# PolyChord/PolyChordLite

Hardware: AMD Instinct MI355X
Metric: likelihood evals/sec, 20D Gaussian nlive=2000 (higher is better)
Workload: dtype f64; 1 GPU; configs[1]: 20-D Gaussian, nlive=2000, num_repeats=40, one full run per step; batch_chains=1000, parallelism=repeat-sharded x1, mode=one run at a time per GPU; R runs in step: roofline.in_step

## Files before the change

include/polychord_hip.h:

```cpp
#ifndef POLYCHORD_HIP_H
#define POLYCHORD_HIP_H
#include <stdbool.h>
#ifdef __cplusplus
extern "C" {
#endif


typedef double (*polychord_loglike_fn)(double *theta, int nDims, double *phi, int nDerived);
typedef void (*polychord_prior_fn)(double *cube, double *theta, int nDims);
typedef void (*polychord_dumper_fn)(int ndead, int nlive, int npars, double *live, double *dead,
                                    double *logweights, double logZ, double logZerr);

void polychord_c_interface(
    polychord_loglike_fn loglikelihood, polychord_prior_fn prior, polychord_dumper_fn dumper,
    int nlive, int num_repeats, int nprior, int nfail, bool do_clustering, int feedback,
    double precision_criterion, double logzero, int max_ndead, double boost_posterior,
    bool posteriors, bool equals, bool cluster_posteriors, bool write_resume, bool write_paramnames,
    bool read_resume, bool write_stats, bool write_live, bool write_dead, bool write_prior,
    bool maximise, double compression_factor, bool synchronous, int nDims, int nDerived,
    char *base_dir, char *file_root, int nGrade, double *grade_frac, int *grade_dims, int n_nlives,
    double *loglikes, int *nlives, int seed, int *comm);

void polychord_c_interface_ini(polychord_loglike_fn loglikelihood, void (*setup_loglikelihood)(void),
                               char *inifile, int *comm);
// ... 229 lines not shown
int  pchip_run_in_step(const pchip_settings *s, const pchip_like *like, const pchip_prior *prior, int nseeds, const int *seeds,
                       int ndevices, const int *devices, int max_in_flight, int want_rows, pchip_result *results, pchip_merged *merged);

typedef struct pchip_comm pchip_comm;
#define PCHIP_COMM_ID_BYTES 128
int  pchip_comm_get_id(char *id128);
int  pchip_comm_create(const char *id128, int nranks, int rank, int device, pchip_comm **out);
void pchip_comm_destroy(pchip_comm *c);
int  pchip_comm_merge(pchip_comm *c, const pchip_result *run, double logzero, int nDims, int nDerived, int want_rows,
                      pchip_merged *out);
int  pchip_comm_merge_many(pchip_comm *c, const pchip_result *runs, int nruns, double logzero, int nDims, int nDerived, int want_rows,
                           pchip_merged *out);
typedef int (*pchip_allgather_fn)(void *user, const void *send, void *recv, unsigned long bytes);
int  pchip_comm_create_with(pchip_allgather_fn all_gather, void *user, int nranks, int rank, int device, pchip_comm **out);
const char *pchip_comm_library(void);

int  pchip_slice_chains(const pchip_settings *s, const pchip_like *like, const pchip_prior *prior,
                        unsigned batch, int nchains, const double *seeds, const double *chol,
                        double contour, double *babies_out, double *nhats_out, int *nlike_out);
#define PCHIP_NO_SUCH_PATH 64
int  pchip_directions(const pchip_settings *s, const pchip_like *like, const pchip_prior *prior, unsigned batch, int nchains,
                      const double *seeds, const double *chol, int path, double *nhat_out, double *nhat_w_out,
                      double *nhat_Ms_out, double *ch_My_out, int *has_Ms, double *raw_out, int nrows, int nbases);
int  pchip_prior_transform(const pchip_prior *prior, int nDims, int n, const double *cube, double *theta, int device);
int  pchip_update_factors(const pchip_settings *s, int ncluster, int nlive, const double *live, const int *live_cluster,
                          int nph, const double *phantom, const double *ph_logL, const int *ph_cluster, const double *threshold,
                          const double *shift, int path, double *cov, double *chol, int *count, double *shift_out, int *chol_suspect);
typedef struct {
    int ncluster, nlive, nph;
    const double *live, *live_logL; const int *live_cluster;
    const double *phantom, *ph_logL; const int *ph_cluster;
} pchip_cluster_in;
typedef struct {
    int maxc, nsplit_cap, scratch_cap;
    int ncluster, nsplit, levels, scratch_n;
    int *live_cluster, *live_pos, *cl_list;
    int *cl_n, *imin_slot, *ph_count; unsigned *cl_uid;
    double *logLp, *lse_ref, *lse_sum, *logXp, *logZp, *logZXp, *logZp2, *logZpXp;
    double *XpXq;
    int *ph_cluster;
    unsigned *split_child, *split_parent; double *split_logfrac;
    double *init;
    double *scratch_Sm; int *scratch_knn, *scratch_lab;
} pchip_cluster_out;
int  pchip_cluster_update(const pchip_settings *s, int nsets, const pchip_cluster_in *in, pchip_cluster_out *out, int path);

// ... 12 lines not shown
```

polychordlite_amd/_ctypes_api.py:

```python
import ctypes as C
import os

import numpy as np

_HERE = os.path.dirname(os.path.abspath(__file__))
LIB_PATH = os.environ.get("PCHIP_LIB") or os.path.join(_HERE, "libpolychord_hip.so")

LOGLIKE_FN = C.CFUNCTYPE(C.c_double, C.POINTER(C.c_double), C.c_int, C.POINTER(C.c_double), C.c_int)
PRIOR_FN = C.CFUNCTYPE(None, C.POINTER(C.c_double), C.POINTER(C.c_double), C.c_int)
DUMPER_FN = C.CFUNCTYPE(None, C.c_int, C.c_int, C.c_int, C.POINTER(C.c_double), C.POINTER(C.c_double),
                        C.POINTER(C.c_double), C.c_double, C.c_double)

LIKE_CALLBACK, LIKE_GAUSSIAN, LIKE_RASTRIGIN, LIKE_TWIN_GAUSSIAN, LIKE_CORR_GAUSSIAN, LIKE_SOURCE = range(6)
KERNEL_CLASSES = ("k_nhats", "k_slice", "k_consume", "k_apply", "k_clean", "k_covmats", "k_bases_side")
LIKE_KINDS = {"gaussian": LIKE_GAUSSIAN, "rastrigin": LIKE_RASTRIGIN, "twin_gaussian": LIKE_TWIN_GAUSSIAN,
              "corr_gaussian": LIKE_CORR_GAUSSIAN, "source": LIKE_SOURCE}


class Settings(C.Structure):
    _fields_ = [("nDims", C.c_int), ("nDerived", C.c_int), ("nlive", C.c_int), ("num_repeats", C.c_int),
                ("nprior", C.c_int), ("nfail", C.c_int), ("do_clustering", C.c_int),
                ("precision_criterion", C.c_double), ("logzero", C.c_double), ("max_ndead", C.c_int),
                ("boost_posterior", C.c_double), ("posteriors", C.c_int), ("equals", C.c_int),
                ("cluster_posteriors", C.c_int), ("compression_factor", C.c_double), ("n_nlives", C.c_int),
# ... 474 lines not shown
    ch = np.ascontiguousarray(chol, dtype=np.float64)
    assert ch.shape == (D, D) and sd.shape[1] == 2 * D + settings.nDerived + 2
    nch = sd.shape[0]
    if settings.nGrade > 1:
        off = np.concatenate([[0], np.cumsum([settings.grade_dims[g] for g in range(settings.nGrade)])[:-1]])
        reps = [settings.grade_repeats[g] for g in range(settings.nGrade)]
    else:
        off, reps = [0], [settings.num_repeats]
    nr = int(sum(reps))
    nb = int(sum(-(-r // (D - o)) for r, o in zip(reps, off)))
    nhat = np.full((nch, nr, D), np.nan); w = np.full((nch, nr), np.nan)
    Ms = np.full((nch, nr, D), np.nan); My = np.full((nch, D), np.nan); raw = np.full((nch, nb, D, D), np.nan)
    has = C.c_int(0)
    rc = lib.pchip_directions(C.byref(settings), C.byref(like), C.byref(prior), batch, nch, dptr(sd), dptr(ch), path, dptr(nhat), dptr(w),
                              dptr(Ms), dptr(My), C.byref(has), dptr(raw), nr, nb)
    if rc == NO_SUCH_PATH:
        return None
    if rc != 0:
        msg = lib.polychord_hip_last_error()
        raise RuntimeError(f"pchip_directions failed with code {rc}" + (": " + msg.decode(errors="replace") if rc == 1 and msg else ""))
    return dict(nhat=nhat, nhat_w=w, nhat_Ms=Ms if has.value else None, ch_My=My if has.value else None, raw=raw if path else None)


def maximum_dict(m, nDims, nDerived):
    n = nDims + nDerived
    pt = lambda p: np.ctypeslib.as_array(p, shape=(n,)).copy() if p else None
    return dict(status=[int(v) for v in m.status], cluster=[int(v) for v in m.cluster], niter=[int(v) for v in m.niter], neval=[int(v) for v in m.neval],
                max_logl=m.max_logl, max_point=pt(m.max_point), max_post=m.max_post, logl_at_post=m.logl_at_post, post_point=pt(m.post_point),
                logl_mean=m.logl_mean if m.has_mean else None, mean_point=pt(m.mean_point) if m.has_mean else None)


def _maximum_out(lib, m, rc, who, nDims, nDerived, write):
    try:
        if rc != 0 and not (rc == 1 and m.max_point and (m.status[0] or m.status[1])):
            msg = lib.polychord_hip_last_error()
            raise RuntimeError(f"{who} failed with code {rc}" + (": " + msg.decode(errors="replace") if msg else ""))
        if write is not None and lib.pchip_maximum_write(C.byref(m), nDims, nDerived, str(write).encode()) != 0:
            raise RuntimeError(f"pchip_maximum_write({write}) failed")
        return maximum_dict(m, nDims, nDerived)
    finally:
        lib.pchip_maximum_free(C.byref(m))


def maximise_device(settings, like, prior, run, max_iter=0, write=None):
    lib = load()
    live = np.ascontiguousarray(run["live"], dtype=np.float64)
# ... 129 lines not shown
```

polychordlite_amd/csrc/pc_dev.h:

```cpp
#pragma once
#ifndef __HIPCC_RTC__
#include <hip/hip_runtime.h>
#include <stdint.h>
#else
using __hip_internal::uint32_t; using __hip_internal::uint64_t; using __hip_internal::int32_t; using __hip_internal::int64_t;
typedef unsigned long uintptr_t;
#endif

#define PC_WAVE 64
#define PC_SLICE_STRIDE 128
enum { PC_DOM_LIVEGEN = 0, PC_DOM_SEED = 1, PC_DOM_NHAT = 2, PC_DOM_SHUFFLE = 3, PC_DOM_SLICE = 4,
       PC_DOM_PHANTOM = 5, PC_DOM_POST = 6, PC_DOM_SEQ = 0xFFFF };
enum { PC_LIKE_CALLBACK = 0, PC_LIKE_GAUSSIAN = 1, PC_LIKE_RASTRIGIN = 2, PC_LIKE_TWIN_GAUSSIAN = 3,
       PC_LIKE_CORR_GAUSSIAN = 4, PC_LIKE_SOURCE = 5 };
#define PC_SRC_MAX_DERIVED 32

#define PC_HUGE 1.7976931348623157e308
#define PC_LOG_TWO_PI 1.8378770664093453
#define PC_TWO_PI 6.283185307179586

struct u32x4 { uint32_t x, y, z, w; };

__device__ __forceinline__ u32x4 philox4x32_10(uint32_t c0, uint32_t c1, uint32_t c2, uint32_t c3,
                                                uint32_t k0, uint32_t k1)
// ... 96 lines not shown
__device__ inline double pc_inv_normal_tail(double p)
{
    const double c[8] = { 1.42343711074968357734e+00, 4.63033784615654529590e+00,
        5.76949722146069140550e+00, 3.64784832476320460504e+00, 1.27045825245236838258e+00,
        2.41780725177450611770e-01, 2.27238449892691845833e-02, 7.74545014278341407640e-04 };
    const double d[8] = { 1.0, 2.05319162663775882187e+00, 1.67638483018380384940e+00,
        6.89767334985100004550e-01, 1.48103976427480074590e-01, 1.51986665636164571966e-02,
        5.47593808499534494600e-04, 1.05075007164441684324e-09 };
    const double e[8] = { 6.65790464350110377720e+00, 5.46378491116411436990e+00,
        1.78482653991729133580e+00, 2.96560571828504891230e-01, 2.65321895265761230930e-02,
        1.24266094738807843860e-03, 2.71155556874348757815e-05, 2.01033439929228813265e-07 };
    const double f[8] = { 1.0, 5.99832206555887937690e-01, 1.36929880922735805310e-01,
        1.48753612908506148525e-02, 7.86869131145613259100e-04, 1.84631831751005468180e-05,
        1.42151175831644588870e-07, 2.04426310338993978564e-15 };
    const double q = p - 0.5;
    double r = (q < 0.0) ? p : 1.0 - p;
    r = sqrt(-log(r));
    double v;
    if (r <= 5.0) { r -= 1.6; v = poly8(c, r) / poly8(d, r); }
    else          { r -= 5.0; v = poly8(e, r) / poly8(f, r); }
    return (q < 0.0) ? -v : v;
}

__device__ __forceinline__ double pc_logaddexp(double a, double b)
{
    const bool ab = a > b;
    const double hi = ab ? a : b, d = ab ? b - a : a - b;
    if (d < -37.0) return hi;
    return hi + log(exp(d) + 1.0);
}

__device__ __forceinline__ void pc_lds_barrier() { asm volatile("s_waitcnt lgkmcnt(0)\n\ts_barrier" ::: "memory"); }

#define PC_DPP_XOR1 0xB1
#define PC_DPP_XOR2 0x4E
#define PC_DPP_HALF_MIRROR 0x141
#define PC_DPP_MIRROR 0x140
template <int CTRL>
constexpr bool pc_dpp_full = CTRL < 0x100 || CTRL == PC_DPP_HALF_MIRROR || CTRL == PC_DPP_MIRROR;
template <int CTRL>
__device__ __forceinline__ int dpp_i32(int v) { return __builtin_amdgcn_update_dpp(0, v, CTRL, 0xF, 0xF, pc_dpp_full<CTRL>); }
template <int CTRL>
__device__ __forceinline__ double dpp_f64(double v)
{
    const int lo = dpp_i32<CTRL>(__double2loint(v));
    const int hi = dpp_i32<CTRL>(__double2hiint(v));
// ... 98 lines not shown
```

polychordlite_amd/csrc/pc_engine.hip:

```cpp
#include "pc_state.h"
#include "pc_resume.h"
#include "pc_prior_table.h"
#include "pc_launch.h"
#include "pc_plan.h"
#include <cstdio>
#include <cstdlib>
#include <cstring>
#include <cstdarg>
#include <cstdint>
#include <new>
#include <cmath>
#include <vector>
#include <memory>
#include <string>
#include <chrono>
#include <algorithm>
#include <map>
#include <unordered_map>
#include <atomic>
#include <mutex>
#include <thread>
#include <functional>
#include <exception>
#include <ucontext.h>
// ... 1601 lines not shown
    }
    bool enqueue_nursery()
    {
        unsigned &batch = r_batch; int &nursery_left = r_nursery_left;
        if (S.pool) {
            if (pool_cursor + (long long)B * S.nr > S.Pcap) pool_compact();
            S.pool_base = (int)pool_cursor; S.pool_rows = B * S.nr; S.babies = S.phantom + (size_t)pool_cursor * S.nT;
            pool_cursor += (long long)B * S.nr;
        }
        {
            hipEvent_t e0 = kt.begin(KT_NHATS);
            const PcNurseryChoice ch = pc_choose_nursery(plan, nursery_facts(batch));
            pc_count(path, ch);
            pc_count_step(path, ch);
            int bases_seq = 0;
            switch (ch.bases) {
            case PC_BASES_READY: case PC_BASES_PART1: case PC_BASES_PART1_STEP: {
                RawSlot &rs = ring[batch % raw_depth];
                S.nhat_raw = raw_buf[batch % raw_depth];
                if (ch.bases == PC_BASES_READY) { if (!rs.waited) HIPCHK(hipStreamWaitEvent(st, rs.ready, 0)); bases_seq = rs.co_seq; }
                else {
                    if (rs.valid) HIPCHK(hipStreamWaitEvent(st, rs.ready, 0));
                    if (ch.bases == PC_BASES_PART1_STEP) co->rec(rec_bases(S, batch, B));
                    else (void)pc_launch_nhats_part(&S, batch, B, 1, st, ch.packed ? 1 : 0);
                }
                rs.valid = false;
                if (ch.part2) { if (co) { co->flush(); co->wait_next(); } (void)pc_launch_nhats_part(&S, batch, B, 2, st, 0); }
                break;
            }
            case PC_BASES_NHATS_G: co->rec(rec_nhats_g(S, batch, B)); break;
            case PC_BASES_WHOLE:
                if (co) co->flush();
                if (pc_launch_nhats(&S, batch, B, st)) { std::fprintf(stderr, "polychord_hip: nDims unsupported\n"); r_rc = 3; return false; }
                break;
            }
            kt.end(KT_NHATS, e0);
            hipEvent_t e1 = kt.begin(KT_SLICE);
            switch (ch.sampler) {
            case PC_SAMPLER_CALLBACK:
                if (co) co->flush();
                if (dev_batch) slice_device(batch); else slice_callback(batch);
                if (stop.load(std::memory_order_relaxed)) { r_rc = 5; return false; }
                break;
            case PC_SAMPLER_LANE: { Cohort::Rec r = rec_slice(S, batch, B, bases_seq); r.note = co ? &step_note : nullptr; (void)stage(r); break; }
            case PC_SAMPLER_WAVE_STEP: co->rec(rec_slice_g(S, batch, B, ch.fused, ch.fused ? bases_seq : 0, &step_note)); break;
            case PC_SAMPLER_WAVE:
                if (co) { co->flush(); co->wait_next(); }
// ... 39 lines not shown
        if (!ev_presort_a) { ev_presort_a = hpool().get_sync_event(); ev_presort_b = hpool().get_sync_event(); }
        HIPCHK(hipEventRecord(ev_presort_a, st)); HIPCHK(hipStreamWaitEvent(st_side, ev_presort_a, 0));
        if (pc_launch_sort_live(&S, st_side) != 0) return;
        HIPCHK(hipEventRecord(ev_presort_b, st_side));
        presorted = true;
    }
    void side_prefetch(unsigned cur)
    {
        const unsigned batch = cur;
        {
        ensure_side();
        const bool side_free = pc_env().side_free || (S.D > 64 && !pc_env().side_ordered);
        RawSlot &cur = ring[batch % raw_depth];
        if (side_free) { HIPCHK(hipEventRecord(cur.consumed, st)); cur.used = true; }
        if (!side_free) { HIPCHK(hipEventRecord(ev_main, st)); HIPCHK(hipStreamWaitEvent(st_side, ev_main, 0)); }
        const unsigned xmax = batch + (unsigned)raw_depth - (side_free ? 0u : 1u);
        for (unsigned x = batch + 1; x <= xmax; ++x) {
            RawSlot &rs = ring[x % raw_depth];
            if (rs.valid && rs.batch == x && rs.B == B) continue;
            if (rs.valid) continue;
            if (rs.used) HIPCHK(hipStreamWaitEvent(st_side, rs.consumed, 0));
            PcState S1 = S; S1.nhat_raw = raw_buf[x % raw_depth];
            hipEvent_t es = kt.begin_on(KT_SIDE, st_side);
            (void)pc_launch_nhats_part(&S1, x, B, 1, st_side, (cfg.ablate & PC_ABL_BASES_PACKED) ? 1 : 0);
            kt.end_on(KT_SIDE, es, st_side);
            HIPCHK(hipEventRecord(rs.ready, st_side));
            rs.valid = true; rs.batch = x; rs.B = B; rs.waited = false;
        }
    }
    }

    PcContractFacts contract_facts(int nursery_left) const
    {
        PcContractFacts f{};
        f.ncluster = h_ctl->ncluster; f.nursery_left = nursery_left;
        f.in_step = co != nullptr; f.cohort_general = cohort_general_ok();
        f.nn_lists = S.nn_list && !pc_env().nn_lists_off; f.nn_valid = S.nn_valid != 0;
        f.cl_fits = f.ncluster > 1 && pc_consume_cl_fits(&S, f.ncluster) != 0;
        f.clp_fits = f.cl_fits && pc_consume_clp_fits(&S, f.ncluster) != 0;
        return f;
    }
    bool round_enqueue()
    {
        unsigned &batch = r_batch; bool &sort_valid = r_sort_valid; int &nursery_left = r_nursery_left;
        {
            if (h_ctl->status == PC_ST_DONE) return false;
            if (h_ctl->status == PC_ST_ERROR) { std::fprintf(stderr, "polychord_hip: device error %d\n", h_ctl->error); r_rc = 2; return false; }
// ... 431 lines not shown
    try {
        E.setup(c, *like, *prior);
        PcState &S = E.S;
        const int nT = S.nT, D = S.D, nr = S.nr, nb = S.nb_total;
        if (nrows != nr || nbases != nb) {
            pc_abi_set_last_error("pchip_directions: the caller's arrays are for another number of directions or bases than the settings give");
            rc = 1;
        } else if ((path != 0 && !pc_nhats_splittable(&S)) || (path == 2 && !pc_bases_t_ok(&S))) rc = PCHIP_NO_SUCH_PATH;
        if (has_Ms) *has_Ms = S.nhat_Ms != nullptr ? 1 : 0;
        if (rc == 0) {
            HIPCHK(hipMemcpy(S.live, seeds, sizeof(double) * (size_t)nchains * nT, hipMemcpyHostToDevice));
            std::vector<double> ll(nchains); std::vector<int> idn(nchains), zero(nchains, 0);
            for (int i = 0; i < nchains; ++i) { ll[i] = seeds[(size_t)i * nT + S.l0]; idn[i] = i; }
            const double contour = *std::min_element(ll.begin(), ll.end());
            HIPCHK(hipMemcpy(S.live_logL, ll.data(), sizeof(double) * nchains, hipMemcpyHostToDevice));
            HIPCHK(hipMemcpy(S.live_cluster, zero.data(), sizeof(int) * nchains, hipMemcpyHostToDevice));
            HIPCHK(hipMemcpy(S.live_pos, idn.data(), sizeof(int) * nchains, hipMemcpyHostToDevice));
            HIPCHK(hipMemcpy(S.cl_list, idn.data(), sizeof(int) * nchains, hipMemcpyHostToDevice));
            HIPCHK(hipMemcpy(S.cl_n, &nchains, sizeof(int), hipMemcpyHostToDevice));
            HIPCHK(hipMemcpy(S.logLp, &contour, sizeof(double), hipMemcpyHostToDevice));
            HIPCHK(hipMemcpy(S.chol, chol, sizeof(double) * D * D, hipMemcpyHostToDevice));
            S.seed_override = 1;
            if (path == 0) rc = pc_launch_nhats(&S, batch, nchains, E.st) ? PCHIP_NO_SUCH_PATH : 0;
            else rc = (pc_launch_nhats_part(&S, batch, nchains, 1, E.st, path == 2 ? 1 : 0) || pc_launch_nhats_part(&S, batch, nchains, 2, E.st, 0)) ? PCHIP_NO_SUCH_PATH : 0;
            HIPCHK(hipStreamSynchronize(E.st));
            HIPCHK(hipGetLastError());
        }
        if (rc == 0) {
            HIPCHK(hipMemcpy(nhat_out, S.nhat, sizeof(double) * (size_t)nchains * nr * D, hipMemcpyDeviceToHost));
            HIPCHK(hipMemcpy(nhat_w_out, S.nhat_w, sizeof(double) * (size_t)nchains * nr, hipMemcpyDeviceToHost));
            if (S.nhat_Ms && nhat_Ms_out) HIPCHK(hipMemcpy(nhat_Ms_out, S.nhat_Ms, sizeof(double) * (size_t)nchains * nr * D, hipMemcpyDeviceToHost));
            if (S.ch_My && ch_My_out) HIPCHK(hipMemcpy(ch_My_out, S.ch_My, sizeof(double) * (size_t)nchains * D, hipMemcpyDeviceToHost));
        }
        if (rc == 0 && path != 0) {
            const size_t blk = D <= 24 ? (size_t)D * D : D <= 32 ? (size_t)1024 : D <= 64 ? (size_t)4096 : (size_t)32 * 512;
            std::vector<double> raw((size_t)nchains * nb * blk);
            HIPCHK(hipMemcpy(raw.data(), S.nhat_raw, sizeof(double) * raw.size(), hipMemcpyDeviceToHost));
            for (size_t cb = 0; cb < (size_t)nchains * nb; ++cb) {
                const double *in = raw.data() + cb * blk;
                double *out = raw_out + cb * (size_t)D * D;
                for (int v = 0; v < D; ++v)
                    for (int d = 0; d < D; ++d) {
                        size_t at;
                        if (D <= 24) at = (size_t)v * D + d;
                        else if (D <= 64) at = (size_t)v * (D <= 32 ? 32 : 64) + d;
                        else { const int n = 2 * (d >> 3) + (d & 1), lk = (d & 7) >> 1; at = (size_t)n * 512 + 64 * (v >> 4) + 16 * lk + (v & 15); }
                        out[(size_t)v * D + d] = in[at];
                    }
            }
        }
    } catch (const EngineError &e) {
        std::fprintf(stderr, "polychord_hip: %s\n", e.msg.c_str());
        (void)hipGetLastError();
        rc = e.code;
    }
    E.destroy();
    return rc;
}

int pchip_prior_transform(const pchip_prior *prior, int nDims, int n, const double *cube, double *theta, int device)
{
    if (!prior || prior->kind != PCHIP_PRIOR_TABLE || n < 1 || !cube || !theta) { pc_abi_set_last_error("pchip_prior_transform: a prior table (kind 2) and n >= 1 points"); return 1; }
    PcPriorTable T;
    const std::string err = pc_prior_table_build(nDims, prior->table, prior->hyper, T);
    if (!err.empty()) { pc_abi_set_last_error(err.c_str()); return 1; }
    if (nDims > 256) return 3;
    int ndev = 0;
    if (hipGetDeviceCount(&ndev) != hipSuccess || ndev == 0) { (void)hipGetLastError(); std::fprintf(stderr, "polychord_hip: no HIP device available -- this engine has no CPU path\n"); return 2; }
    if (hipSetDevice(device >= 0 ? device % ndev : 0) != hipSuccess) return 2;
    const std::vector<double> tp = T.dev_par(); const std::vector<int> ti = T.dev_int();
    double *d_tp = nullptr, *d_c = nullptr, *d_t = nullptr; int *d_ti = nullptr;
    const size_t nb = sizeof(double) * (size_t)n * nDims;
// ... 605 lines not shown
```

polychordlite_amd/csrc/pc_launch.h:

```cpp
#pragma once
#include "pc_state.h"
#include "../../include/polychord_hip.h"
#include <cstddef>
#include <memory>
#include <vector>

struct PcSourceForm {
    long nterms;
    int nsums;
    long nquad;
    long nshared;
    int has_prior;
    long long ndata, ntail;
    int alive;
};

static inline size_t pc_quad_lds(const PcSourceForm &f) { return f.nquad > 0 ? sizeof(double) * 2 * (size_t)((f.nquad + 1) & ~1L) : 0; }

static inline size_t pc_front_lds(const PcSourceForm &f) { return pc_quad_lds(f) + (f.nshared > 0 ? sizeof(double) * 2 * (size_t)((f.nshared + 1) & ~1L) : 0); }

static inline int pc_slice_phi_lds(const PcState *S, const PcSourceForm &f)
{
    const size_t sh0 = sizeof(double) * ((size_t)S->D + S->nr) + 16, tb = sizeof(double) * (size_t)S->nr * (S->D + 1);
    const size_t sums = sizeof(double) * (size_t)S->nr * (size_t)f.nsums;
// ... 61 lines not shown
void pc_batch_callback_get(polychord_batch_fn *fn, void **user);
int pc_device_batch_registered(void);
int pc_fast_fits(const PcState *S);
int pc_launch_sort_live(const PcState *S, hipStream_t st);
int pc_launch_sort_live_many(const PcState *S, const PcManyRec *dR, int R, hipStream_t st);
int pc_launch_consume_fast(const PcState *S, int final_mode, hipStream_t st);
void pc_launch_ph_prepare(const PcState *S, hipStream_t st);
size_t pc_records_block_bytes(long long cap, int nT);
int pc_pack_lived_device(const double *dead, const double *logw, const double *entry, long long nd, int nT, double logzero, double *block, long long cap, long long *h_count, hipStream_t st);
int pc_par_fits(const PcState *S);
int pc_launch_consume_par(const PcState *S, hipStream_t st);
int pc_launch_consume_par_many(const PcState *S, const PcManyRec *dR, int R, hipStream_t st);
int pc_launch_par_accept(int n, const double *snap, int T, const double *cand, const unsigned char *valid, int serial, unsigned char *accept,
                         hipStream_t st);
int pc_launch_final_par(const PcState *S, hipStream_t st);
int pc_launch_final_par_split(const PcState *S, hipStream_t st);
int pc_launch_final_par_many(const PcManyRec *dR, int R, hipStream_t st);
int pc_rtc_launch(const PcState *S, const char *expr, dim3 grid, dim3 block, size_t sh, hipStream_t st, void **args);
const char *pc_rtc_error(void);
int pc_rtc_source_form(int id, PcSourceForm *f);
int pc_rtc_wanted(const PcState *S);
int pc_launch_generate_live(const PcState *S, int attempt0, int n, double *rows, double *rows_logL, hipStream_t st);
int pc_nhats_splittable(const PcState *S);
int pc_launch_nhats_part(const PcState *S, unsigned batch, int nchains, int part, hipStream_t st, int packed);
int pc_launch_nhats(const PcState *S, unsigned batch, int nchains, hipStream_t st);
int pc_slice_fusable(const PcState *S);
int pc_launch_slice_fused(const PcState *S, unsigned batch, int nchains, hipStream_t st);
int pc_launch_slice_many(const PcState *S, const PcManyRec *dR, int R, int nchains, int fused, hipStream_t st);
int pc_launch_slice_step(const PcState *S, const PcManyRec *dR, int R, int nchains, int fused, hipStream_t st);
int pc_launch_nhats_many(const PcState *S, const PcManyRec *dR, int R, int nchains, hipStream_t st);
int pc_launch_slice(const PcState *S, unsigned batch, int nchains, hipStream_t st);
int pc_launch_prior_transform(const PcState *S, int n, const double *cubes, double *thetas, hipStream_t st);
int pc_launch_source_eval(const PcState *S, int n, const double *thetas, double *logL, double *phi, hipStream_t st);
int pc_launch_source_prior_eval(const PcState *S, int n, const double *cubes, double *thetas, hipStream_t st);
int pc_launch_max_rank(const PcState *S, int n, const double *rows, double *val, hipStream_t st);
int pc_launch_maximise(const PcState *S, int nprob, const double *in, const int *hdr, long long max_iter, double *out, long long *outi, hipStream_t st);
int pc_max_choose_simplex(int nDims, int nTotal, double logzero, const double *live, const int *cluster, int nlive, const double *vals,
                          double *simplex, double *f);
void pc_maximum_alloc(pchip_maximum *m, int nDims, int nDerived);
int pc_bases_t_ok(const PcState *S);
int pc_launch_bases_t(const PcState *S, unsigned batch, int nchains, hipStream_t st);
int pc_launch_bases_t_many(const PcState *S, const PcManyRec *dR, int R, unsigned batch, int nchains, hipStream_t st);
int pc_slice_t_ok(const PcState *S, int ncluster);
int pc_launch_slice_t(const PcState *S, unsigned batch, int nchains, hipStream_t st);
int pc_launch_slice_t_many(const PcState *S, const PcManyRec *dR, int R, unsigned batch, int nchains, hipStream_t st);
int pc_update_fused_ok(const PcState *S, int nc);
// ... 14 lines not shown
```

polychordlite_amd/csrc/pc_sample.hip:

```cpp
#include "pc_state.h"
#ifndef __HIPCC_RTC__
#include <cstdlib>
#endif

template <int DPL>
struct LaneDims {
    double lo[DPL], span[DPL];
    double mean[DPL];
    bool on[DPL];
};

__device__ __forceinline__ double pc_box_theta(double lo, double span, double cube) { return lo + span * cube; }
#define PC_PT_SORTED (1u << 16)
#define PC_PT_PERMUTED (1u << 17)
#define PC_PT_ADAPTIVE (1u << 18)
#define PC_PT_LAYER (1u << 19)
template <int DPL>
struct LaneTable {
    int type[DPL], pos[DPL], len[DPL], hyp[DPL];
    int cnt[DPL], lay[DPL];
    double p0[DPL], p1[DPL], p2[DPL];
    unsigned mask;
};
template <int DPL, bool AD>
// ... 1141 lines not shown
        if (active && wanted) {
            double n0 = 0.0, n1 = 0.0;
            int d = 0;
            for (; d + 1 < D; d += 2) { n0 += mine[d] * mine[d]; n1 += mine[d + 1] * mine[d + 1]; }
            if (d < D) n0 += mine[d] * mine[d];
            const double w = sqrt(n0 + n1);
            Q[i] = 1.0 / w;
            S.nhat_w[(size_t)chain * nr + col] = w * 3.0;
        }
        __syncthreads();
        for (int r = 0; r < Dg && basis * Dg + r < nrg; ++r) {
            double *out = S.nhat + ((size_t)chain * nr + col0 + basis * Dg + r) * D;
            const double iw = Q[r];
            for (int d = tid; d < D; d += NT) out[d] = G[(size_t)r * DS + d] * iw;
        }
    }
#ifdef NHATS_DBG
    ncyc[5] = clock64();
    if (tid == 0 && blockIdx.x == 0 && blockIdx.y == 0) for (int x = 0; x < 5; ++x) S.ctl->dbg[x] += ncyc[x + 1] - ncyc[x];
#endif
#undef PC_DOT4
}

#define PC_BIG_NT 256
#define PC_BIG_P 16
__global__ __launch_bounds__(PC_BIG_NT) void k_nhats_big(PcState S, unsigned batch)
{
    __shared__ int sh[2];
    __shared__ double iwv[PC_BIG_NT];
    __shared__ double Pq[PC_BIG_P * PC_BIG_NT];
    __shared__ double pqq[PC_BIG_P];
    const int D = S.D, nr = S.nr, tid = threadIdx.x, chain = blockIdx.y, i = tid;
    int grade, basis;
    pc_grade_of_basis(S, blockIdx.x, grade, basis);
    const int off = pc_sel(S.g_off, grade), Dg = D - off, nrg = pc_sel(S.g_nr, grade), col0 = pc_sel(S.g_col0, grade);
    if (tid == 0) {
        int sel, slot;
        select_seed(S, batch, chain, sel, slot);
        sh[0] = sel; sh[1] = slot;
        if (blockIdx.x == 0) {
            S.ch_cluster[chain] = sel; S.ch_seed_slot[chain] = slot;
            S.ch_contour[chain] = S.logLp[sel];
            S.ch_epoch[chain] = S.ctl->admin_epoch;
            if (chain == 0) { S.ctl->i_nursery = gridDim.y; S.ctl->batch_id = batch; }
        }
    }
// ... 772 lines not shown
{
    const size_t sh = sizeof(double) * S->D + pc_front_lds(pc_state_form(S));
    const bool table = S->prior.kind >= 2;
    switch (pc_dpl(S->D) + (table ? 8 : 0)) {
    case 1: PC_LAUNCH((k_generate_live<1>), dim3(n), dim3(64), sh, st, *S, attempt0, rows, rows_logL); return 0;
    case 2: PC_LAUNCH((k_generate_live<2>), dim3(n), dim3(64), sh, st, *S, attempt0, rows, rows_logL); return 0;
    case 4: PC_LAUNCH((k_generate_live<4>), dim3(n), dim3(64), sh, st, *S, attempt0, rows, rows_logL); return 0;
    case 9: PC_LAUNCH((k_generate_live<1, 1>), dim3(n), dim3(64), sh, st, *S, attempt0, rows, rows_logL); return 0;
    case 10: PC_LAUNCH((k_generate_live<2, 1>), dim3(n), dim3(64), sh, st, *S, attempt0, rows, rows_logL); return 0;
    case 12: PC_LAUNCH((k_generate_live<4, 1>), dim3(n), dim3(64), sh, st, *S, attempt0, rows, rows_logL); return 0;
    }
    return 1;
}

extern "C" int pc_nhats_splittable(const PcState *S)
{
    const char *e = std::getenv("PC_NHATS_QUAD_MIN");
    if (S->D > 64 && S->D <= 128) return S->ngrade <= 1 && !S->seq_mode && S->nhat_raw != nullptr;
    if (S->D > 24 && S->D <= 64) return S->ngrade <= 1 && !S->seq_mode && S->nhat_raw != nullptr && (!e || std::atoi(e) <= 25);
    return S->D <= 24 && S->D < (e ? std::atoi(e) : 25) && !S->seq_mode && S->nhat_raw != nullptr;
}
static size_t pc_nhats_q_lds(int HV) { return sizeof(double) * (size_t)(2 + HV) * 4 * (HV + 2); }
static size_t pc_nhats_q32_lds(int D) { const int NR = ((D + 15) / 16) * 16; return sizeof(double) * (2 * 4 * 34 + (size_t)(NR + (NR <= 112 ? 32 : 16)) * 129); }
extern "C" int pc_launch_nhats_part(const PcState *S, unsigned batch, int nchains, int part, hipStream_t st, int packed)
{
    if (!pc_nhats_splittable(S)) return 1;
    const int D = S->D;
    dim3 grid(S->nb_total, nchains);
    if (D > 64) {
        if (part == 1) {
            static const bool panel_off = std::getenv("PC_BASIS_PANEL_OFF") != nullptr;
            const int nt1 = (D + 15) / 16;
            if (panel_off) hipLaunchKernelGGL((k_nhats_q<32, 1>), grid, dim3(512), sizeof(double) * 2 * 4 * 34, st, *S, batch);
            else if (nt1 <= 5) hipLaunchKernelGGL((k_basis<5>), grid, dim3(512), 0, st, *S, batch);
            else if (nt1 == 6) hipLaunchKernelGGL((k_basis<6>), grid, dim3(512), 0, st, *S, batch);
            else if (nt1 == 7) hipLaunchKernelGGL((k_basis<7>), grid, dim3(512), 0, st, *S, batch);
            else hipLaunchKernelGGL((k_basis<8>), grid, dim3(512), 0, st, *S, batch);
        }
        else {
            dim3 g2(S->nb_total * 2, nchains);
            const int nt = (D + 15) / 16;
            if (nt <= 5) hipLaunchKernelGGL((k_whiten<5>), g2, dim3(256), 0, st, *S, batch);
            else if (nt == 6) hipLaunchKernelGGL((k_whiten<6>), g2, dim3(256), 0, st, *S, batch);
            else if (nt == 7) hipLaunchKernelGGL((k_whiten<7>), g2, dim3(256), 0, st, *S, batch);
            else hipLaunchKernelGGL((k_whiten<8>), g2, dim3(256), 0, st, *S, batch);
        }
        return 0;
    }
    if (D > 24) {
        if (D <= 32) { if (part == 1) hipLaunchKernelGGL((k_nhats_q<8, 1>), grid, dim3(128), pc_nhats_q_lds(8), st, *S, batch); else hipLaunchKernelGGL((k_nhats_q<8, 2>), grid, dim3(128), pc_nhats_q_lds(8), st, *S, batch); }
        else { if (part == 1) hipLaunchKernelGGL((k_nhats_q<16, 1>), grid, dim3(256), pc_nhats_q_lds(16), st, *S, batch); else hipLaunchKernelGGL((k_nhats_q<16, 2>), grid, dim3(256), pc_nhats_q_lds(16), st, *S, batch); }
        return 0;
    }
    const size_t sh = sizeof(double) * ((size_t)(D + 8) * (D + 8) + 2 * 128) + 16;
    if (part == 1 && packed && pc_launch_bases_t(S, batch, nchains, st) == 0) return 0;
    if (part == 1) {
        if (D <= 8) hipLaunchKernelGGL((k_nhats<8, 64, 1>), grid, dim3(64), sh, st, *S, batch);
        else if (D <= 16) hipLaunchKernelGGL((k_nhats<16, 64, 1>), grid, dim3(64), sh, st, *S, batch);
        else hipLaunchKernelGGL((k_nhats<24, 64, 1>), grid, dim3(64), sh, st, *S, batch);
    } else {
        if (D <= 8) hipLaunchKernelGGL((k_nhats<8, 64, 2>), grid, dim3(64), sh, st, *S, batch);
        else if (D <= 16) hipLaunchKernelGGL((k_nhats<16, 64, 2>), grid, dim3(64), sh, st, *S, batch);
        else hipLaunchKernelGGL((k_nhats<24, 64, 2>), grid, dim3(64), sh, st, *S, batch);
    }
    return 0;
}

extern "C" int pc_launch_nhats(const PcState *S, unsigned batch, int nchains, hipStream_t st)
{
    const int D = S->D, nb = S->nb_total;
    dim3 grid(nb, nchains);
    static int quad_min = -1;
    if (quad_min < 0) { const char *e = std::getenv("PC_NHATS_QUAD_MIN"); quad_min = e ? std::atoi(e) : 25; }
    if (D >= quad_min) {
        if (D <= 32) hipLaunchKernelGGL((k_nhats_q<8>), grid, dim3(128), pc_nhats_q_lds(8), st, *S, batch);
        else if (D <= 64) hipLaunchKernelGGL((k_nhats_q<16>), grid, dim3(256), pc_nhats_q_lds(16), st, *S, batch);
        else if (D <= 128) {
            const size_t shq = pc_nhats_q32_lds(D);
// ... 249 lines not shown
```

polychordlite_amd/csrc/pc_slice_t.hip:

```cpp
#include "pc_state.h"
#include "pc_launch.h"
#include <cstdlib>

namespace {

struct Q3 { double a, b, c; };

template <int D>
struct TriMap {
    int aa[D * (D + 1) / 2], bb[D * (D + 1) / 2];
    constexpr TriMap() : aa{}, bb{} { int e = 0; for (int b = 0; b < D; ++b) for (int a = b; a < D; ++a) { aa[e] = a; bb[e] = b; ++e; } }
};

template <int DT, int LO, int N, class F>
__device__ __forceinline__ Q3 tree3(const F &leaf)
{
#pragma clang fp contract(off)
    if constexpr (LO >= DT) return Q3{0.0, 0.0, 0.0};
    else if constexpr (N == 1) return leaf(LO);
    else {
        const Q3 l = tree3<DT, LO, N / 2>(leaf);
        if constexpr (LO + N / 2 >= DT && N / 2 >= 16) return l;
        const Q3 r = tree3<DT, LO + N / 2, N / 2>(leaf);
        return Q3{l.a + r.a, l.b + r.b, l.c + r.c};
// ... 405 lines not shown
    const bool unit = S->prior.lo == nullptr && S->prior.hi == nullptr;
    static const bool help_off = std::getenv("PC_SLICE_T_HELP_OFF") != nullptr;
    static const long long help_env = std::getenv("PC_SLICE_T_HELP_MAX") ? std::atoll(std::getenv("PC_SLICE_T_HELP_MAX")) : -1;
    const long long help_max = help_env >= 0 ? help_env : 256LL * std::max<long long>(1, std::min<long long>(2, (long long)(156 * 1024) / (long long)shh));
    const bool help = dR && !help_off && shh <= 64 * 1024 && (long long)grid * R <= help_max;
    const size_t lds = help ? shh : sh;
#define PC_T_MANY(UNIT, HELP) { \
        if (lds > 48 * 1024) pc_need_dyn_lds((const void *)k_slice_t_many<DT, UNIT, HELP>, lds); \
        hipLaunchKernelGGL((k_slice_t_many<DT, UNIT, HELP>), dim3(grid, R), dim3(HELP ? 192 : 64), lds, st, dR, nchains, nrp); }
#define PC_T_ONE(UNIT) { \
        if (lds > 48 * 1024) pc_need_dyn_lds((const void *)k_slice_t<DT, UNIT>, lds); \
        hipLaunchKernelGGL((k_slice_t<DT, UNIT>), dim3(grid), dim3(64), lds, st, *S, batch, nchains, nrp); }
    if (help) { if (unit) PC_T_MANY(true, true) else PC_T_MANY(false, true) }
    else if (dR) { if (unit) PC_T_MANY(true, false) else PC_T_MANY(false, false) }
    else { if (unit) PC_T_ONE(true) else PC_T_ONE(false) }
#undef PC_T_ONE
#undef PC_T_MANY
}

}

namespace {

template <int D, bool FIRST_RIGHT>
__device__ __forceinline__ double dot4_same(const double (&a)[D])
{
#pragma clang fp contract(off)
    double pp[4];
#pragma unroll
    for (int k = 0; k < 4; ++k) {
        if (k >= D) pp[k] = 0.0;
        else if (k + 4 >= D) pp[k] = fma(a[k], a[k], 0.0);
        else if (FIRST_RIGHT && k == 0) pp[k] = fma(a[k + 4 < D ? k + 4 : 0], a[k + 4 < D ? k + 4 : 0], a[k] * a[k]);
        else pp[k] = fma(a[k], a[k], a[k + 4 < D ? k + 4 : 0] * a[k + 4 < D ? k + 4 : 0]);
    }
#pragma unroll
    for (int d = 8; d < D; ++d) pp[d & 3] = fma(a[d], a[d], pp[d & 3]);
    return (pp[0] + pp[1]) + (pp[2] + pp[3]);
}
template <int D>
__device__ __forceinline__ double dot4(const double (&a)[D], const double (&b)[D])
{
#pragma clang fp contract(off)
    double pp[4] = {0.0, 0.0, 0.0, 0.0};
#pragma unroll
    for (int d = 0; d < D; ++d) pp[d & 3] = fma(a[d], b[d], pp[d & 3]);
    return (pp[0] + pp[1]) + (pp[2] + pp[3]);
}

template <int DMAX>
__device__ __forceinline__ void bases_packed_body(const PcState &S, int nbases)
{
#pragma clang fp contract(off)
    extern __shared__ __attribute__((aligned(16))) char smem[];
    const int D = S.D, per = 64 / D;
    const int tid = threadIdx.x, sub = tid / D, i = tid - sub * D;
    const int g = blockIdx.x * per + sub;
    const bool active = sub < per && g < nbases;
    double *Q = (double *)smem + (size_t)(sub < per ? sub : 0) * 2 * DMAX;
    double v[DMAX];
    double *raw = S.nhat_raw + ((size_t)(active ? g : 0) * D + i) * D;
#pragma unroll
    for (int d = 0; d < DMAX; ++d) v[d] = (active && d < D) ? raw[d] : 0.0;
    {
        const double inrm = 1.0 / sqrt(dot4_same<DMAX, (DMAX <= 16)>(v));
#pragma unroll
        for (int d = 0; d < DMAX; ++d) v[d] = v[d] * inrm;
    }
    if (i == 0 && active) {
#pragma unroll
        for (int d = 0; d < DMAX; ++d) Q[d] = v[d];
    }
    __syncthreads();
    for (int j = 0; j < D; ++j) {
        const double *q = Q + (size_t)(j & 1) * DMAX;
        double qv[DMAX];
#pragma unroll
        for (int d = 0; d < DMAX; ++d) qv[d] = active ? q[d] : 0.0;
        const double qq = dot4_same<DMAX, false>(qv), dv = dot4<DMAX>(qv, v);
        if (i == j) {
            const double inrm = 1.0 / sqrt(qq);
#pragma unroll
            for (int d = 0; d < DMAX; ++d) v[d] = v[d] * inrm;
        } else if (active && i > j) {
            const double cproj = dv / qq;
#pragma unroll
            for (int d = 0; d < DMAX; ++d) v[d] = fma(-cproj, qv[d], v[d]);
            if (i == j + 1) {
                double *qn = Q + (size_t)((j + 1) & 1) * DMAX;
#pragma unroll
                for (int d = 0; d < DMAX; ++d) qn[d] = v[d];
            }
        }
        __syncthreads();
    }
    if (active) {
#pragma unroll
        for (int d = 0; d < DMAX; ++d) if (d < D) raw[d] = v[d];
    }
}
template <int DMAX>
__global__ __launch_bounds__(64) void k_bases_packed(PcState S, int nbases) { bases_packed_body<DMAX>(S, nbases); }
template <int DMAX>
__global__ __launch_bounds__(64) void k_bases_packed_many(const PcManyRec *R, int nbases) { bases_packed_body<DMAX>(pc_many_state(R, blockIdx.y), nbases); }

#define DEVT_CALLS 4
__device__ __forceinline__ void deviates_t_body(const PcState &S, unsigned batch, int nbases, int NC)
{
    __shared__ double qU[4][2 * DEVT_CALLS * 64];
    __shared__ int qA[4][2 * DEVT_CALLS * 64];
    const int D = S.D, DD = D * D, lane = threadIdx.x & 63, wv = threadIdx.x >> 6;
    const long long ncalls = (long long)nbases * NC;
    int qn = 0;
    auto put = [&](bool want, double u, int dst) {
        bool t = false;
        double x = 0.0;
        if (want) x = pc_inv_normal_central(u, t);
        if (want && !t) S.nhat_raw[dst] = x;
// ... 90 lines not shown
```

polychordlite_amd/csrc/pc_state.h:

```cpp
#pragma once
#include "pc_dev.h"

enum { PC_ST_RUNNING = 0, PC_ST_DONE = 1, PC_ST_UPDATE = 2, PC_ST_ERROR = 4 };
enum { PC_ERR_NONE = 0, PC_ERR_PHANTOM_CAP = 1, PC_ERR_DEAD_CAP = 2, PC_ERR_CLUSTER_CAP = 3, PC_ERR_NOSLOT = 4 };

enum { PC_ABL_FUNCTOR = 1 << 0, PC_ABL_NO_POOL = 1 << 1, PC_ABL_NO_DEFER = 1 << 2, PC_ABL_NO_FUSED_UPDATE = 1 << 3, PC_ABL_PAIR_SCANS = 1 << 4,
       PC_ABL_CONSUME_GENERAL = 1 << 5, PC_ABL_SLICE_LANE = 1 << 6, PC_ABL_BASES_PACKED = 1 << 7, PC_ABL_CL_END_AT_DEATH = 1 << 8,
       PC_ABL_KILLOFF_GENERAL = 1 << 9, PC_ABL_CONSUME_CL_SERIAL = 1 << 10, PC_ABL_RETIRED_11 = 1 << 11, PC_ABL_RETIRED_12 = 1 << 12,
       PC_ABL_NO_HELPER = 1 << 13, PC_ABL_QC_BY_CHAIN = 1 << 14, PC_ABL_RTC_BUILTINS = 1 << 15, PC_ABL_UPDATE_CHAIN = 1 << 16, PC_ABL_FLAG_LAUNCH = 1 << 17,
       PC_ABL_ACCEPT_SERIAL = 1 << 18, PC_ABL_TRACE_CHOL = 1 << 30 };

#define PC_MASK_WORDS 16

struct PcCtl {
    int status;
    int error;
    int i_nursery;
    int admin_epoch;
    int failures;
    int ncluster;
    int ncluster_dead;
    int ndead;
    int nphantom;
    int seg_hi, seg_lo;
    int cluster_deleted;
    unsigned batch_id;
    unsigned next_cluster_uid;
    long long nlike;
    long long niter;
    long long nlike_device;
    long long nlike_failed;
    double logZ, logZ2;
    double logX_last_update;
// ... 227 lines not shown
```

Before: 1.392 billion likelihood evals/s.

## Fuse nhat random generation and Gram-Schmidt into one wave-per-bases kernel

Adds k_nhats_w, which draws the Gaussian deviates for several bases straight into shared memory, resolves tail inverse-normal cases through a compacted queue, and runs the packed Gram-Schmidt on them in the same 64-thread block. It becomes the default part-1 path, replacing the generic k_nhats part-1 kernel unless the new ablation bit is set. The aim is to avoid the separate raw-deviate write and re-read and to raise occupancy through small packed blocks. The Gram-Schmidt body is moved into a shared macro, and a deck_records test entry point is added. It risks divergence in the ballot queue and adds extra record writes for the deck.

```diff
diff --git a/include/polychord_hip.h b/include/polychord_hip.h
--- a/include/polychord_hip.h
+++ b/include/polychord_hip.h
@@ -275,6 +275,7 @@
 int  pchip_directions(const pchip_settings *s, const pchip_like *like, const pchip_prior *prior, unsigned batch, int nchains,
                       const double *seeds, const double *chol, int path, double *nhat_out, double *nhat_w_out,
                       double *nhat_Ms_out, double *ch_My_out, int *has_Ms, double *raw_out, int nrows, int nbases);
+int  pchip_deck_records(const pchip_settings *s, const pchip_like *like, const pchip_prior *prior, unsigned batch, int nchains, int *records);
 int  pchip_prior_transform(const pchip_prior *prior, int nDims, int n, const double *cube, double *theta, int device);
 int  pchip_update_factors(const pchip_settings *s, int ncluster, int nlive, const double *live, const int *live_cluster,
                           int nph, const double *phantom, const double *ph_logL, const int *ph_cluster, const double *threshold,
diff --git a/polychordlite_amd/_ctypes_api.py b/polychordlite_amd/_ctypes_api.py
--- a/polychordlite_amd/_ctypes_api.py
+++ b/polychordlite_amd/_ctypes_api.py
@@ -520,6 +520,20 @@
     return dict(nhat=nhat, nhat_w=w, nhat_Ms=Ms if has.value else None, ch_My=My if has.value else None, raw=raw if path else None)
 
 
+def deck_records(settings, like, prior, batch, nchains, fill=-1):
+    lib = load()
+    lib.pchip_deck_records.argtypes = [C.POINTER(Settings), C.POINTER(Like), C.POINTER(Prior), C.c_uint, C.c_int, C.POINTER(C.c_int)]
+    lib.pchip_deck_records.restype = C.c_int
+    rec = np.full((nchains, 66), fill, dtype=np.int32)
+    rc = lib.pchip_deck_records(C.byref(settings), C.byref(like), C.byref(prior), batch, nchains, rec.ctypes.data_as(C.POINTER(C.c_int)))
+    if rc == NO_SUCH_PATH:
+        return None
+    if rc != 0:
+        msg = lib.polychord_hip_last_error()
+        raise RuntimeError(f"pchip_deck_records failed with code {rc}" + (": " + msg.decode(errors="replace") if rc == 1 and msg else ""))
+    return rec
+
+
 def maximum_dict(m, nDims, nDerived):
     n = nDims + nDerived
     pt = lambda p: np.ctypeslib.as_array(p, shape=(n,)).copy() if p else None
diff --git a/polychordlite_amd/csrc/pc_dev.h b/polychordlite_amd/csrc/pc_dev.h
--- a/polychordlite_amd/csrc/pc_dev.h
+++ b/polychordlite_amd/csrc/pc_dev.h
@@ -142,6 +142,59 @@
     return (q < 0.0) ? -v : v;
 }
 
+template <int D, bool FIRST_RIGHT>
+__device__ __forceinline__ double dot4_same(const double (&a)[D])
+{
+#pragma clang fp contract(off)
+    double pp[4];
+#pragma unroll
+    for (int k = 0; k < 4; ++k) {
+        if (k >= D) pp[k] = 0.0;
+        else if (k + 4 >= D) pp[k] = fma(a[k], a[k], 0.0);
+        else if (FIRST_RIGHT && k == 0) pp[k] = fma(a[k + 4 < D ? k + 4 : 0], a[k + 4 < D ? k + 4 : 0], a[k] * a[k]);
+        else pp[k] = fma(a[k], a[k], a[k + 4 < D ? k + 4 : 0] * a[k + 4 < D ? k + 4 : 0]);
+    }
+#pragma unroll
+    for (int d = 8; d < D; ++d) pp[d & 3] = fma(a[d], a[d], pp[d & 3]);
+    return (pp[0] + pp[1]) + (pp[2] + pp[3]);
+}
+template <int D>
+__device__ __forceinline__ double dot4(const double (&a)[D], const double (&b)[D])
+{
+#pragma clang fp contract(off)
+    double pp[4] = {0.0, 0.0, 0.0, 0.0};
+#pragma unroll
+    for (int d = 0; d < D; ++d) pp[d & 3] = fma(a[d], b[d], pp[d & 3]);
+    return (pp[0] + pp[1]) + (pp[2] + pp[3]);
+}
+#define PC_GS_PACKED(DMAX, v, Q, D, i, active) \
+    {    \
+        const double inrm = 1.0 / sqrt(dot4_same<DMAX, (DMAX <= 16)>(v)); \
+        _Pragma("unroll") for (int d = 0; d < DMAX; ++d) v[d] = v[d] * inrm; \
+    } \
+    if (i == 0 && active) { \
+        _Pragma("unroll") for (int d = 0; d < DMAX; ++d) Q[d] = v[d]; \
+    } \
+    __syncthreads(); \
+    for (int j = 0; j < D; ++j) {                                                \
+        const double *q = Q + (size_t)(j & 1) * DMAX; \
+        double qv[DMAX]; \
+        _Pragma("unroll") for (int d = 0; d < DMAX; ++d) qv[d] = active ? q[d] : 0.0; \
+        const double qq = dot4_same<DMAX, false>(qv), dv = dot4<DMAX>(qv, v); \
+        if (i == j) { \
+            const double inrm = 1.0 / sqrt(qq); \
+            _Pragma("unroll") for (int d = 0; d < DMAX; ++d) v[d] = v[d] * inrm; \
+        } else if (active && i > j) { \
+            const double cproj = dv / qq; \
+            _Pragma("unroll") for (int d = 0; d < DMAX; ++d) v[d] = fma(-cproj, qv[d], v[d]); \
+            if (i == j + 1) { \
+                double *qn = Q + (size_t)((j + 1) & 1) * DMAX; \
+                _Pragma("unroll") for (int d = 0; d < DMAX; ++d) qn[d] = v[d]; \
+            } \
+        } \
+        __syncthreads(); \
+    }
+
 __device__ __forceinline__ double pc_logaddexp(double a, double b)
 {
     const bool ab = a > b;
diff --git a/polychordlite_amd/csrc/pc_engine.hip b/polychordlite_amd/csrc/pc_engine.hip
--- a/polychordlite_amd/csrc/pc_engine.hip
+++ b/polychordlite_amd/csrc/pc_engine.hip
@@ -1647,7 +1647,7 @@
                 else {
                     if (rs.valid) HIPCHK(hipStreamWaitEvent(st, rs.ready, 0));
                     if (ch.bases == PC_BASES_PART1_STEP) co->rec(rec_bases(S, batch, B));
-                    else (void)pc_launch_nhats_part(&S, batch, B, 1, st, ch.packed ? 1 : 0);
+                    else (void)pc_launch_nhats_part(&S, batch, B, 1, st, pc_part1_kind(ch.packed, cfg.ablate));
                 }
                 rs.valid = false;
                 if (ch.part2) { if (co) { co->flush(); co->wait_next(); } (void)pc_launch_nhats_part(&S, batch, B, 2, st, 0); }
@@ -1733,7 +1733,7 @@
             if (rs.used) HIPCHK(hipStreamWaitEvent(st_side, rs.consumed, 0));
             PcState S1 = S; S1.nhat_raw = raw_buf[x % raw_depth];
             hipEvent_t es = kt.begin_on(KT_SIDE, st_side);
-            (void)pc_launch_nhats_part(&S1, x, B, 1, st_side, (cfg.ablate & PC_ABL_BASES_PACKED) ? 1 : 0);
+            (void)pc_launch_nhats_part(&S1, x, B, 1, st_side, pc_part1_kind((cfg.ablate & PC_ABL_BASES_PACKED) != 0, cfg.ablate));
             kt.end_on(KT_SIDE, es, st_side);
             HIPCHK(hipEventRecord(rs.ready, st_side));
             rs.valid = true; rs.batch = x; rs.B = B; rs.waited = false;
@@ -2211,7 +2211,7 @@
             HIPCHK(hipMemcpy(S.chol, chol, sizeof(double) * D * D, hipMemcpyHostToDevice));
             S.seed_override = 1;
             if (path == 0) rc = pc_launch_nhats(&S, batch, nchains, E.st) ? PCHIP_NO_SUCH_PATH : 0;
-            else rc = (pc_launch_nhats_part(&S, batch, nchains, 1, E.st, path == 2 ? 1 : 0) || pc_launch_nhats_part(&S, batch, nchains, 2, E.st, 0)) ? PCHIP_NO_SUCH_PATH : 0;
+            else rc = (pc_launch_nhats_part(&S, batch, nchains, 1, E.st, pc_part1_kind(path == 2, c.ablate)) || pc_launch_nhats_part(&S, batch, nchains, 2, E.st, 0)) ? PCHIP_NO_SUCH_PATH : 0;
             HIPCHK(hipStreamSynchronize(E.st));
             HIPCHK(hipGetLastError());
         }
@@ -2237,6 +2237,42 @@
                         out[(size_t)v * D + d] = in[at];
                     }
             }
+        }
+    } catch (const EngineError &e) {
+        std::fprintf(stderr, "polychord_hip: %s\n", e.msg.c_str());
+        (void)hipGetLastError();
+        rc = e.code;
+    }
+    E.destroy();
+    return rc;
+}
+
+int pchip_deck_records(const pchip_settings *s, const pchip_like *like, const pchip_prior *prior, unsigned batch, int nchains, int *records_out)
+{
+    if (!s || !like || !prior || nchains < 1 || !records_out) {
+        pc_abi_set_last_error("pchip_deck_records: settings, likelihood, prior, nchains >= 1 and an array of 66 ints a chain");
+        return 1;
+    }
+    if (like->kind == PCHIP_LIKE_SOURCE || (s->ablate & PC_ABL_RTC_BUILTINS)) {
+        pc_abi_set_last_error("pchip_deck_records does not take a device source likelihood (or settings.ablate bit 15)");
+        return 1;
+    }
+    if (s->nDims > 24) return PCHIP_NO_SUCH_PATH;
+    pchip_settings c = *s;
+    c.nlive = nchains; c.nprior = nchains; c.batch = nchains; c.do_clustering = 0;
+    Engine E;
+    int rc = 0;
+    try {
+        E.setup(c, *like, *prior);
+        PcState &S = E.S;
+        if (!pc_nhats_splittable(&S) || S.ngrade > 1) rc = PCHIP_NO_SUCH_PATH;
+        else {
+            int *rec = (int *)(S.nhat_raw + (size_t)S.B * S.nb_total * S.D * S.D);
+            HIPCHK(hipMemcpy(rec, records_out, sizeof(int) * (size_t)nchains * 66, hipMemcpyHostToDevice));
+            rc = pc_launch_nhats_part(&S, batch, nchains, 1, E.st, pc_part1_kind(false, c.ablate)) ? PCHIP_NO_SUCH_PATH : 0;
+            HIPCHK(hipStreamSynchronize(E.st));
+            HIPCHK(hipGetLastError());
+            if (rc == 0) HIPCHK(hipMemcpy(records_out, rec, sizeof(int) * (size_t)nchains * 66, hipMemcpyDeviceToHost));
         }
     } catch (const EngineError &e) {
         std::fprintf(stderr, "polychord_hip: %s\n", e.msg.c_str());
diff --git a/polychordlite_amd/csrc/pc_launch.h b/polychordlite_amd/csrc/pc_launch.h
--- a/polychordlite_amd/csrc/pc_launch.h
+++ b/polychordlite_amd/csrc/pc_launch.h
@@ -107,6 +107,10 @@
 int pc_rtc_wanted(const PcState *S);
 int pc_launch_generate_live(const PcState *S, int attempt0, int n, double *rows, double *rows_logL, hipStream_t st);
 int pc_nhats_splittable(const PcState *S);
+enum { PC_PART1_BASIS = 0,
+       PC_PART1_PACKED = 1,
+       PC_PART1_WAVE = 2 };
+static inline int pc_part1_kind(bool packed, int ablate) { return packed ? PC_PART1_PACKED : ((ablate & PC_ABL_BASES_WAVE) ? PC_PART1_BASIS : PC_PART1_WAVE); }
 int pc_launch_nhats_part(const PcState *S, unsigned batch, int nchains, int part, hipStream_t st, int packed);
 int pc_launch_nhats(const PcState *S, unsigned batch, int nchains, hipStream_t st);
 int pc_slice_fusable(const PcState *S);
diff --git a/polychordlite_amd/csrc/pc_sample.hip b/polychordlite_amd/csrc/pc_sample.hip
--- a/polychordlite_amd/csrc/pc_sample.hip
+++ b/polychordlite_amd/csrc/pc_sample.hip
@@ -1187,6 +1187,71 @@
 #undef PC_DOT4
 }
 
+template <int DMAX>
+__global__ __launch_bounds__(64) void k_nhats_w(PcState S, unsigned batch, int nbases)
+{
+    extern __shared__ __attribute__((aligned(16))) char smem[];
+    const int D = S.D, DD = D * D, nb = S.nb_total, nr = S.nr, per = 64 / D, NC = (DD + 1) / 2;
+    const int tid = threadIdx.x, sub = tid / D, i = tid - sub * D;
+    const int g0 = blockIdx.x * per, g = g0 + sub;
+    const int nbw = nbases - g0 < per ? nbases - g0 : per;
+    const bool active = sub < per && g < nbases;
+    double *G = (double *)smem;
+    double *Qw = G + (size_t)per * DD;
+    int *qA = (int *)(Qw + (size_t)per * 2 * DMAX);
+    if (nr <= 64) {
+        for (int s = 0; s < nbw; ++s) {
+            const int chain = (g0 + s) / nb;
+            if (g0 + s != chain * nb) continue;
+            const int dk = pc_deck_keyed(S, batch, chain, tid, nr);
+            int *rec = pc_deck_record(S, chain);
+            rec[2 + tid] = dk;
+            const unsigned long long tg = pc_deck_tag(S, batch, chain, nr);
+            if (tid == 0) { rec[0] = (int)(unsigned)tg; rec[1] = (int)(unsigned)(tg >> 32); }
+        }
+    }
+    int qn = 0;
+    auto put = [&](bool want, double u, int dst) {
+        bool t = false;
+        double x = 0.0;
+        if (want) x = pc_inv_normal_central(u, t);
+        if (want) G[dst] = t ? u : x;
+        const unsigned long long m = __ballot(want && t);
+        if (want && t) qA[qn + __popcll(m & ((1ull << tid) - 1ull))] = dst;
+        qn += __popcll(m);
+    };
+    for (int t0 = 0; t0 < nbw * NC; t0 += 64) {
+        const int t = t0 + tid;
+        const bool in = t < nbw * NC;
+        const int s = in ? t / NC : 0, m = in ? t - s * NC : 0;
+        const int chain = (g0 + s) / nb, basis = (g0 + s) - chain * nb;
+        const uint32_t e0 = (uint32_t)pc_sel(S.g_e0, 0) + (uint32_t)basis * DD, e1 = e0 + (uint32_t)DD;
+        const uint32_t call = (e0 >> 1) + (uint32_t)m;
+        double ua = 0.5, ub = 0.5;
+        if (in) pc_uniform2(S.k0, S.k1, PC_DOM_NHAT, batch, (uint32_t)chain, call, ua, ub);
+        const uint32_t ia = 2 * call, ib = ia + 1;
+        put(in && ia >= e0 && ia < e1, ua, s * DD + (int)(ia - e0));
+        put(in && ib >= e0 && ib < e1, ub, s * DD + (int)(ib - e0));
+    }
+    __syncthreads();
+    for (int k = tid; k < qn; k += 64) { const int at = qA[k]; G[at] = pc_inv_normal_tail(G[at]); }
+    __syncthreads();
+    double v[DMAX];
+    const double *mine = G + (size_t)(active ? sub : 0) * DD + (size_t)i * D;
+#pragma unroll
+    for (int d = 0; d < DMAX; ++d) v[d] = (active && d < D) ? mine[d] : 0.0;
+    double *Q = Qw + (size_t)(sub < per ? sub : 0) * 2 * DMAX;
+    {
+#pragma clang fp contract(off)
+        PC_GS_PACKED(DMAX, v, Q, D, i, active)
+    }
+    if (active) {
+        double *raw = S.nhat_raw + ((size_t)g * D + i) * D;
+#pragma unroll
+        for (int d = 0; d < DMAX; ++d) if (d < D) raw[d] = v[d];
+    }
+}
+
 #define PC_BIG_NT 256
 #define PC_BIG_P 16
 __global__ __launch_bounds__(PC_BIG_NT) void k_nhats_big(PcState S, unsigned batch)
@@ -2005,6 +2070,7 @@
 }
 static size_t pc_nhats_q_lds(int HV) { return sizeof(double) * (size_t)(2 + HV) * 4 * (HV + 2); }
 static size_t pc_nhats_q32_lds(int D) { const int NR = ((D + 15) / 16) * 16; return sizeof(double) * (2 * 4 * 34 + (size_t)(NR + (NR <= 112 ? 32 : 16)) * 129); }
+static size_t pc_nhats_w_lds(int D, int DMAX) { return (size_t)(64 / D) * (sizeof(double) * ((size_t)D * D + 2 * DMAX) + sizeof(int) * (size_t)D * D); }
 extern "C" int pc_launch_nhats_part(const PcState *S, unsigned batch, int nchains, int part, hipStream_t st, int packed)
 {
     if (!pc_nhats_splittable(S)) return 1;
@@ -2036,7 +2102,15 @@
         return 0;
     }
     const size_t sh = sizeof(double) * ((size_t)(D + 8) * (D + 8) + 2 * 128) + 16;
-    if (part == 1 && packed && pc_launch_bases_t(S, batch, nchains, st) == 0) return 0;
+    if (part == 1 && packed == PC_PART1_PACKED && pc_launch_bases_t(S, batch, nchains, st) == 0) return 0;
+    if (part == 1 && packed == PC_PART1_WAVE && S->ngrade <= 1) {
+        const int nbases = nchains * S->nb_total, per = 64 / D;
+        const dim3 gw((nbases + per - 1) / per);
+        if (D <= 8) hipLaunchKernelGGL((k_nhats_w<8>), gw, dim3(64), pc_nhats_w_lds(D, 8), st, *S, batch, nbases);
+        else if (D <= 16) hipLaunchKernelGGL((k_nhats_w<16>), gw, dim3(64), pc_nhats_w_lds(D, 16), st, *S, batch, nbases);
+        else hipLaunchKernelGGL((k_nhats_w<24>), gw, dim3(64), pc_nhats_w_lds(D, 24), st, *S, batch, nbases);
+        return 0;
+    }
     if (part == 1) {
         if (D <= 8) hipLaunchKernelGGL((k_nhats<8, 64, 1>), grid, dim3(64), sh, st, *S, batch);
         else if (D <= 16) hipLaunchKernelGGL((k_nhats<16, 64, 1>), grid, dim3(64), sh, st, *S, batch);
diff --git a/polychordlite_amd/csrc/pc_slice_t.hip b/polychordlite_amd/csrc/pc_slice_t.hip
--- a/polychordlite_amd/csrc/pc_slice_t.hip
+++ b/polychordlite_amd/csrc/pc_slice_t.hip
@@ -451,31 +451,6 @@
 
 namespace {
 
-template <int D, bool FIRST_RIGHT>
-__device__ __forceinline__ double dot4_same(const double (&a)[D])
-{
-#pragma clang fp contract(off)
-    double pp[4];
-#pragma unroll
-    for (int k = 0; k < 4; ++k) {
-        if (k >= D) pp[k] = 0.0;
-        else if (k + 4 >= D) pp[k] = fma(a[k], a[k], 0.0);
-        else if (FIRST_RIGHT && k == 0) pp[k] = fma(a[k + 4 < D ? k + 4 : 0], a[k + 4 < D ? k + 4 : 0], a[k] * a[k]);
-        else pp[k] = fma(a[k], a[k], a[k + 4 < D ? k + 4 : 0] * a[k + 4 < D ? k + 4 : 0]);
-    }
-#pragma unroll
-    for (int d = 8; d < D; ++d) pp[d & 3] = fma(a[d], a[d], pp[d & 3]);
-    return (pp[0] + pp[1]) + (pp[2] + pp[3]);
-}
-template <int D>
-__device__ __forceinline__ double dot4(const double (&a)[D], const double (&b)[D])
-{
-#pragma clang fp contract(off)
-    double pp[4] = {0.0, 0.0, 0.0, 0.0};
-#pragma unroll
-    for (int d = 0; d < D; ++d) pp[d & 3] = fma(a[d], b[d], pp[d & 3]);
-    return (pp[0] + pp[1]) + (pp[2] + pp[3]);
-}
 
 template <int DMAX>
 __device__ __forceinline__ void bases_packed_body(const PcState &S, int nbases)
@@ -491,38 +466,7 @@
     double *raw = S.nhat_raw + ((size_t)(active ? g : 0) * D + i) * D;
 #pragma unroll
     for (int d = 0; d < DMAX; ++d) v[d] = (active && d < D) ? raw[d] : 0.0;
-    {
-        const double inrm = 1.0 / sqrt(dot4_same<DMAX, (DMAX <= 16)>(v));
-#pragma unroll
-        for (int d = 0; d < DMAX; ++d) v[d] = v[d] * inrm;
-    }
-    if (i == 0 && active) {
-#pragma unroll
-        for (int d = 0; d < DMAX; ++d) Q[d] = v[d];
-    }
-    __syncthreads();
-    for (int j = 0; j < D; ++j) {
-        const double *q = Q + (size_t)(j & 1) * DMAX;
-        double qv[DMAX];
-#pragma unroll
-        for (int d = 0; d < DMAX; ++d) qv[d] = active ? q[d] : 0.0;
-        const double qq = dot4_same<DMAX, false>(qv), dv = dot4<DMAX>(qv, v);
-        if (i == j) {
-            const double inrm = 1.0 / sqrt(qq);
-#pragma unroll
-            for (int d = 0; d < DMAX; ++d) v[d] = v[d] * inrm;
-        } else if (active && i > j) {
-            const double cproj = dv / qq;
-#pragma unroll
-            for (int d = 0; d < DMAX; ++d) v[d] = fma(-cproj, qv[d], v[d]);
-            if (i == j + 1) {
-                double *qn = Q + (size_t)((j + 1) & 1) * DMAX;
-#pragma unroll
-                for (int d = 0; d < DMAX; ++d) qn[d] = v[d];
-            }
-        }
-        __syncthreads();
-    }
+    PC_GS_PACKED(DMAX, v, Q, D, i, active)
     if (active) {
 #pragma unroll
         for (int d = 0; d < DMAX; ++d) if (d < D) raw[d] = v[d];
diff --git a/polychordlite_amd/csrc/pc_state.h b/polychordlite_amd/csrc/pc_state.h
--- a/polychordlite_amd/csrc/pc_state.h
+++ b/polychordlite_amd/csrc/pc_state.h
@@ -8,7 +8,7 @@
        PC_ABL_CONSUME_GENERAL = 1 << 5, PC_ABL_SLICE_LANE = 1 << 6, PC_ABL_BASES_PACKED = 1 << 7, PC_ABL_CL_END_AT_DEATH = 1 << 8,
        PC_ABL_KILLOFF_GENERAL = 1 << 9, PC_ABL_CONSUME_CL_SERIAL = 1 << 10, PC_ABL_RETIRED_11 = 1 << 11, PC_ABL_RETIRED_12 = 1 << 12,
        PC_ABL_NO_HELPER = 1 << 13, PC_ABL_QC_BY_CHAIN = 1 << 14, PC_ABL_RTC_BUILTINS = 1 << 15, PC_ABL_UPDATE_CHAIN = 1 << 16, PC_ABL_FLAG_LAUNCH = 1 << 17,
-       PC_ABL_ACCEPT_SERIAL = 1 << 18, PC_ABL_TRACE_CHOL = 1 << 30 };
+       PC_ABL_ACCEPT_SERIAL = 1 << 18, PC_ABL_BASES_WAVE = 1 << 19, PC_ABL_TRACE_CHOL = 1 << 30 };
 
 #define PC_MASK_WORDS 16
 
```

After: 1.419 billion likelihood evals/s (median of 6 runs). 1.9% higher.
